# cts198859/deeprl_signal_control

Hardware: AMD Instinct MI355X
Metric: env-steps/s (agents x envs x sim-steps/s), large_grid MA2C (higher is better)
Workload: dtype f32; 1 GPU; large_grid 5x5 (25 agents), MA2C LSTM policy (neighbour fingerprint gather), 1024 env instances per GPU; step = 120 control steps (x5 sim-steps) of every instance + 1 A2C update (BPTT, clip, RMSProp); envs_per_gpu=1024, n_step=120, agents=25, parallelism=env-sharded x1, live_vehicles=window mean over the timed region

## Files before the change

### deeprl_signal_control_amd/csrc/tsc_model.hip

```cpp
#include "tsc_common.h"
#include "tsc_gemm.h"
#include "../../include/tsc.h"

#include <cstdlib>
#include <type_traits>
#include <vector>

namespace {

using tsc::f32x16;
using tsc::f32x4;
using tsc::GemmArgs;

constexpr int kOut = 8;
constexpr int kL = 64;
constexpr int kG4 = 4 * kL;

struct Layout {
    int G, A, SMAX, AMAX, H;
    int NZ, fc;
    long long stride, oW1, ob1, oWx, oWh, obl, oWo, obo;
};

__device__ __forceinline__ float sigmoidf_(float x) {
// ... 1632 lines not shown

__global__ void rmsprop_kernel(float *w, float *ms, const float *grad, long long per_agent, long long total,
                               const double *norm2, float gscale, float clip, float lr, float alpha, float eps) {
    const long long i = (long long)blockIdx.x * blockDim.x + threadIdx.x;
    if (i >= total) return;
    const int a = (int)(i / per_agent);
    const float nrm = (float)sqrt(norm2[a]);
    float g = grad[i] * gscale;
    if (clip > 0.f) g = g * (clip / fmaxf(nrm, clip));
    const float m = alpha * ms[i] + (1.0f - alpha) * g * g;
    ms[i] = m;
    w[i] = w[i] - lr * g / sqrtf(m + eps);
}

__global__ void transpose_wx_kernel(const float *params, Layout lay, float *WxT) {
    const long long i = (long long)blockIdx.x * blockDim.x + threadIdx.x;
    const long long per = (long long)lay.H * lay.NZ;
    if (i >= per * lay.G) return;
    const int g = (int)(i / per);
    const long long r = i % per;
    const int c = (int)(r / lay.H), h = (int)(r % lay.H);
    WxT[i] = params[(long long)g * lay.stride + lay.oWx + (long long)h * lay.NZ + c];
}

__global__ void interleave_gates_kernel(const float *params, Layout lay, float *Wg) {
    const long long i = (long long)blockIdx.x * blockDim.x + threadIdx.x;
    const long long per = (long long)(lay.H + kL) * kG4;
    if (i >= per * lay.G) return;
    const long long g = i / per, r = i % per;
    const int k = (int)(r / kG4), c = (int)(r % kG4), u = c >> 2, q = c & 3;
    Wg[i] = params[g * lay.stride + lay.oWx + (long long)k * kG4 + 64 * q + u];
}

__global__ void register_order_kernel(const float *params, Layout lay, float *Wr) {
    const long long i = (long long)blockIdx.x * blockDim.x + threadIdx.x;
    const long long per = (long long)(lay.H + kL) * kG4;
    if (i >= per * lay.G) return;
    const long long g = i / per, r = i % per;
    const int c = (int)(r & 3), lane = (int)((r >> 2) & 63);
    const long long rest = r >> 8;
    const int nj = (lay.H + kL) / 8, w = (int)(rest / nj), j4 = (int)(rest % nj);
    const int k = 8 * j4 + 4 * (lane >> 5) + c, col = 32 * w + (lane & 31);
    Wr[i] = params[g * lay.stride + lay.oWx + (long long)k * kG4 + col];
}

__global__ void fill_kernel(float *p, long long n, float v) {
    const long long i = (long long)blockIdx.x * blockDim.x + threadIdx.x;
    if (i < n) p[i] = v;
}

}


template <int NT>
__global__ void __launch_bounds__(512, 1)
dwxh_kernel(const float *__restrict__ X1, const float *__restrict__ Hp, const float *__restrict__ dZ, long long N, int G,
            int S, long long rows_per_split, float *__restrict__ ws) {
    constexpr int HT = NT - 2, H = 32 * HT, KC = 16, LDA = NT * 32 + 4;
    constexpr int XQ = H / 4, NX = KC * XQ, NQ = NX + KC * (kL / 4), NLD = (NQ + 511) / 512;
    __shared__ __attribute__((aligned(16))) float As[2][KC][LDA];
    const int g = blockIdx.x % G, sp = blockIdx.x / G;
    const int tid = threadIdx.x, lane = tid & 63, wave = tid >> 6, li = lane & 31, kh = lane >> 5;
    const int col0 = 32 * wave;
    const long long n0 = (long long)sp * rows_per_split;
    long long n1 = n0 + rows_per_split;
    if (n1 > N) n1 = N;
    const float *x1 = X1 + (long long)g * N * H, *hp = Hp + (long long)g * N * kL;
    const float *dz = dZ + (long long)g * N * kG4 + col0 + li;
    f32x16 acc[NT];
#pragma unroll
    for (int t = 0; t < NT; ++t)
#pragma unroll
        for (int r = 0; r < 16; ++r) acc[t][r] = 0.f;
    float bsum = 0.f;
    static_assert(NLD <= 3, "staging slots");
    struct Slot { int row, col; bool x, ok; };
    auto slot = [&](int q) {
        Slot o;
        int idx = tid + 512 * q;
        o.ok = idx < NQ;
        if (!o.ok) idx = NQ - 1;
        o.x = idx < NX;
        const int j = o.x ? idx : idx - NX, w = o.x ? XQ : kL / 4;
        o.row = j / w; o.col = 4 * (j % w);
        return o;
    };
    const Slot s0 = slot(0), s1 = slot(1), s2 = slot(2);
    float4 g0, g1, g2;
    auto fetch1 = [&](const Slot &o, long long row0) {
        long long row = row0 + o.row;
        if (row >= n1) row = n1 - 1;
        const float *src = o.x ? x1 + row * H + o.col : hp + row * kL + o.col;
        return *reinterpret_cast<const float4 *>(src);
    };
    auto commit1 = [&](const Slot &o, int buf, const float4 &v) {
        if (o.ok) *reinterpret_cast<float4 *>(&As[buf][o.row][(o.x ? 0 : H) + o.col]) = v;
    };
#define DWXH_FETCH(row0) do { g0 = fetch1(s0, row0); if (NLD > 1) g1 = fetch1(s1, row0); if (NLD > 2) g2 = fetch1(s2, row0); } while (0)
#define DWXH_COMMIT(buf) do { commit1(s0, buf, g0); if (NLD > 1) commit1(s1, buf, g1); if (NLD > 2) commit1(s2, buf, g2); } while (0)
    float bcur[KC / 2], bnxt[KC / 2];
    auto fetch_b = [&](float *b, long long row0) {
#pragma unroll
        for (int ks = 0; ks < KC / 2; ++ks) {
            const long long row = row0 + 2 * ks + kh;
            const float z = dz[(row < n1 ? row : n1 - 1) * kG4];
            b[ks] = row < n1 ? z : 0.f;
        }
    };
    if (n0 < n1) {
        DWXH_FETCH(n0); fetch_b(bcur, n0);
        DWXH_COMMIT(0);
        DWXH_FETCH(n0 + KC);
        __syncthreads();
        int buf = 0;
        for (long long row = n0; row < n1; row += KC, buf ^= 1) {
            fetch_b(bnxt, row + KC);
            __builtin_amdgcn_sched_barrier(0);
#pragma unroll
            for (int ks = 0; ks < KC / 2; ++ks) {
                float av[NT];
#pragma unroll
                for (int t = 0; t < NT; ++t) av[t] = As[buf][2 * ks + kh][32 * t + li];
                bsum += bcur[ks];
#pragma unroll
                for (int t = 0; t < NT; ++t) acc[t] = __builtin_amdgcn_mfma_f32_32x32x2f32(av[t], bcur[ks], acc[t], 0, 0, 0);
            }
            __builtin_amdgcn_sched_barrier(0);
            DWXH_COMMIT(buf ^ 1);
            DWXH_FETCH(row + 2 * KC);
#pragma unroll
            for (int ks = 0; ks < KC / 2; ++ks) bcur[ks] = bnxt[ks];
            __syncthreads();
        }
    }
    float *w = ws + ((long long)sp * G + g) * ((long long)(NT * 32 + 1) * kG4);
#pragma unroll
    for (int t = 0; t < NT; ++t)
#pragma unroll
        for (int r = 0; r < 16; ++r) {
            const int row = 32 * t + (r & 3) + 8 * (r >> 2) + 4 * kh;
            w[(long long)row * kG4 + col0 + li] = acc[t][r];
        }
    bsum += __shfl_xor(bsum, 32, 64);
    if (kh == 0) w[(long long)NT * 32 * kG4 + col0 + li] = bsum;
#undef DWXH_FETCH
#undef DWXH_COMMIT
}

__global__ void dwxh_reduce_kernel(const float *__restrict__ ws, int G, int S, long long per, float *__restrict__ grads,
                                   long long stride, long long off) {
    const long long i = (long long)blockIdx.x * blockDim.x + threadIdx.x;
    if (i >= per * G) return;
    const long long g = i / per, j = i % per;
    float acc = 0.f;
    for (int s = 0; s < S; ++s) acc += ws[((long long)s * G + g) * per + j];
    grads[g * stride + off + j] = acc;
}


constexpr int kD1Ld = 260;
constexpr int kObLd = 68;

template <int NCU>
__global__ void __launch_bounds__(512, 1)
dx1w1_kernel2(const float *__restrict__ dZ, const float *__restrict__ X1, const float *__restrict__ WxT,
              const float *__restrict__ obs, long long N, int G, int S, long long rows_per_split, int A, int SMAX,
              float *__restrict__ ws, const int *__restrict__ ftm) {
    constexpr int H = 16 * NCU, NHU = 2 * NCU;
    constexpr int CHI = (NHU + 7) / 8, CLO = NHU / 8;
    static_assert(NHU % 8 == 0 || NHU % 8 == 4, "H must be a multiple of 32");
    extern __shared__ __attribute__((aligned(16))) char smem_raw[];
    float *Az = (float *)smem_raw;
    float *Ob = Az + 2 * 32 * kD1Ld;
    const int g = blockIdx.x % G, sp = blockIdx.x / G, a = g >> 1;
    const int tid = threadIdx.x, lane = tid & 63, wave = __builtin_amdgcn_readfirstlane(tid >> 6), n = lane & 15, kq = lane >> 4;
    const long long n0 = (long long)sp * rows_per_split;
    long long n1 = n0 + rows_per_split;
    if (n1 > N) n1 = N;
    const float *dz = dZ + (long long)g * N * kG4, *x1 = X1 + (long long)g * N * H;
    const long long AS = (long long)A * SMAX;
    const int sq = SMAX >> 2;
    float *w = ws + ((long long)sp * G + g) * ((long long)2 * 65 * H);
    const int st = wave < 4 ? wave * CHI : 4 * CHI + (wave - 4) * CLO, cnt = wave < 4 ? CHI : CLO;
    const int U0 = st >> 1;
    const bool a00 = 2 * U0 >= st, a01 = 2 * U0 + 1 < st + cnt, a10 = 2 * U0 + 2 < st + cnt, a11 = 2 * U0 + 3 < st + cnt;
    const int U1 = U0 + 1 < NCU ? U0 + 1 : NCU - 1;
    const int col0 = 16 * U0 + n, col1 = 16 * U1 + n;
    const int fm0 = ftm[a * NCU + U0], fm1 = ftm[a * NCU + U1];
    float bw0[64], bw1[64];
    {
        const float *src = WxT + (long long)g * kG4 * H + (long long)(4 * kq) * H;
#pragma unroll
        for (int j = 0; j < 16; ++j)
#pragma unroll
            for (int c = 0; c < 4; ++c) {
                bw0[4 * j + c] = src[(long long)(16 * j + c) * H + col0];
                bw1[4 * j + c] = src[(long long)(16 * j + c) * H + col1];
            }
    }
    f32x4 accW[2][4];
#pragma unroll
    for (int u = 0; u < 2; ++u)
#pragma unroll
        for (int ft = 0; ft < 4; ++ft) accW[u][ft] = f32x4{0.f, 0.f, 0.f, 0.f};
    float bsum0 = 0.f, bsum1 = 0.f;
    const int zr = tid >> 6, zc = tid & 63, orow = tid >> 4, oc = tid & 15;
    float4 s0, s1, s2, s3, so;
    auto fetch = [&](long long row0) {
        auto rowc = [&](long long r) { return r < n1 ? r : n1 - 1; };
        s0 = *reinterpret_cast<const float4 *>(dz + rowc(row0 + zr) * kG4 + 4 * zc);
        s1 = *reinterpret_cast<const float4 *>(dz + rowc(row0 + zr + 8) * kG4 + 4 * zc);
        s2 = *reinterpret_cast<const float4 *>(dz + rowc(row0 + zr + 16) * kG4 + 4 * zc);
        s3 = *reinterpret_cast<const float4 *>(dz + rowc(row0 + zr + 24) * kG4 + 4 * zc);
        const float4 o = *reinterpret_cast<const float4 *>(obs + rowc(row0 + orow) * AS + (long long)a * SMAX + 4 * (oc < sq ? oc : 0));
        so = oc < sq ? o : make_float4(0.f, 0.f, 0.f, 0.f);
    };
    auto put = [&](int buf) {
        float *zb = Az + (long long)buf * 32 * kD1Ld + 4 * zc;
        *reinterpret_cast<float4 *>(zb + (zr) * kD1Ld) = s0;
        *reinterpret_cast<float4 *>(zb + (zr + 8) * kD1Ld) = s1;
        *reinterpret_cast<float4 *>(zb + (zr + 16) * kD1Ld) = s2;
        *reinterpret_cast<float4 *>(zb + (zr + 24) * kD1Ld) = s3;
        *reinterpret_cast<float4 *>(Ob + ((long long)buf * 32 + orow) * kObLd + 4 * oc) = so;
    };
    auto unit = [&](int buf, long long row, const float (&bw)[64], int col, bool r0, bool r1, f32x4 (&aw)[4], float &bs, int fm) {
        float xm0[4], xm1[4];
        int zq = 0;
        asm volatile("" : "+v"(zq));
#pragma unroll
        for (int i = 0; i < 4; ++i) {
            long long ra = row + 4 * kq + i + zq, rb = ra + 16;
            if (ra >= n1) ra = n1 - 1;
            if (rb >= n1) rb = n1 - 1;
            xm0[i] = x1[ra * H + col];
            xm1[i] = x1[rb * H + col];
        }
        f32x4 c0 = f32x4{0.f, 0.f, 0.f, 0.f}, c1 = f32x4{0.f, 0.f, 0.f, 0.f};
        const float4 *A0 = reinterpret_cast<const float4 *>(Az + ((long long)buf * 32 + n) * kD1Ld + 4 * kq);
        const float4 *A1 = reinterpret_cast<const float4 *>(Az + ((long long)buf * 32 + 16 + n) * kD1Ld + 4 * kq);
        if (r0 && r1) {
            float4 p = A0[0], q = A1[0];
#pragma unroll
            for (int j = 0; j < 16; ++j) {
                const float4 pn = A0[4 * (j + 1 < 16 ? j + 1 : j)], qn = A1[4 * (j + 1 < 16 ? j + 1 : j)];
                c0 = __builtin_amdgcn_mfma_f32_16x16x4f32(p.x, bw[4 * j], c0, 0, 0, 0);
                c1 = __builtin_amdgcn_mfma_f32_16x16x4f32(q.x, bw[4 * j], c1, 0, 0, 0);
                c0 = __builtin_amdgcn_mfma_f32_16x16x4f32(p.y, bw[4 * j + 1], c0, 0, 0, 0);
                c1 = __builtin_amdgcn_mfma_f32_16x16x4f32(q.y, bw[4 * j + 1], c1, 0, 0, 0);
                c0 = __builtin_amdgcn_mfma_f32_16x16x4f32(p.z, bw[4 * j + 2], c0, 0, 0, 0);
                c1 = __builtin_amdgcn_mfma_f32_16x16x4f32(q.z, bw[4 * j + 2], c1, 0, 0, 0);
                c0 = __builtin_amdgcn_mfma_f32_16x16x4f32(p.w, bw[4 * j + 3], c0, 0, 0, 0);
                c1 = __builtin_amdgcn_mfma_f32_16x16x4f32(q.w, bw[4 * j + 3], c1, 0, 0, 0);
                p = pn; q = qn;
                __builtin_amdgcn_sched_barrier(0);
            }
        } else {
            const float4 *As = r0 ? A0 : A1;
            float4 p = As[0];
#pragma unroll
            for (int j = 0; j < 16; ++j) {
                const float4 pn = As[4 * (j + 1 < 16 ? j + 1 : j)];
                c0 = __builtin_amdgcn_mfma_f32_16x16x4f32(p.x, bw[4 * j], c0, 0, 0, 0);
                c0 = __builtin_amdgcn_mfma_f32_16x16x4f32(p.y, bw[4 * j + 1], c0, 0, 0, 0);
                c0 = __builtin_amdgcn_mfma_f32_16x16x4f32(p.z, bw[4 * j + 2], c0, 0, 0, 0);
                c0 = __builtin_amdgcn_mfma_f32_16x16x4f32(p.w, bw[4 * j + 3], c0, 0, 0, 0);
                p = pn;
                __builtin_amdgcn_sched_barrier(0);
            }
            if (!r0) { c1 = c0; }
        }
        auto tail = [&](int r, const f32x4 &c, const float (&xm)[4]) {
            const float *Os = Ob + ((long long)buf * 32 + 16 * r + 4 * kq) * kObLd + n;
            float os[16];
#pragma unroll
            for (int i = 0; i < 4; ++i)
#pragma unroll
                for (int ft = 0; ft < 4; ++ft) os[4 * ft + i] = Os[i * kObLd + 16 * ft];
            float d[4];
#pragma unroll
            for (int i = 0; i < 4; ++i) {
                d[i] = (xm[i] > 0.f && row + 16 * r + 4 * kq + i < n1) ? c[i] : 0.f;
                bs += d[i];
            }
#pragma unroll
            for (int ft = 0; ft < 4; ++ft)
                if ((fm >> ft) & 1) {
#pragma unroll
                    for (int i = 0; i < 4; ++i) aw[ft] = __builtin_amdgcn_mfma_f32_16x16x4f32(os[4 * ft + i], d[i], aw[ft], 0, 0, 0);
                }
        };
        if (r0) tail(0, c0, xm0);
        if (r1) tail(1, c1, xm1);
    };
    if (n0 < n1) {
        fetch(n0);
        put(0);
        __syncthreads();
        int buf = 0;
        for (long long row = n0; row < n1; row += 32, buf ^= 1) {
            fetch(row + 32);
            if (a00 || a01) unit(buf, row, bw0, col0, a00, a01, accW[0], bsum0, fm0);
            if (a10 || a11) unit(buf, row, bw1, col1, a10, a11, accW[1], bsum1, fm1);
            put(buf ^ 1);
            __syncthreads();
        }
    }
    auto flush = [&](const f32x4 (&aw)[4], float bs, int col, bool r0, bool r1) {
        float *w0 = w + (long long)((r0 ? 0 : 1) * 65) * H;
        float *wz = w + (long long)65 * H;
#pragma unroll
        for (int ft = 0; ft < 4; ++ft)
#pragma unroll
            for (int i = 0; i < 4; ++i) {
                const int f = 16 * ft + 4 * kq + i;
                w0[(long long)f * H + col] = aw[ft][i];
                if (r0 && r1) wz[(long long)f * H + col] = 0.f;
            }
        bs += __shfl_xor(bs, 16, 64);
        bs += __shfl_xor(bs, 32, 64);
        if (kq == 0) {
            w0[(long long)64 * H + col] = bs;
            if (r0 && r1) wz[(long long)64 * H + col] = 0.f;
        }
    };
    if (a00 || a01) flush(accW[0], bsum0, col0, a00, a01);
    if (a10 || a11) flush(accW[1], bsum1, col1, a10, a11);
}

__global__ void dx1w1_reduce2_kernel(const float *__restrict__ ws, int G, int S, int H, int SMAX, const int16_t *__restrict__ rr,
                                     float *__restrict__ grads, long long stride, long long oW1, long long ob1) {
    const long long per = (long long)65 * H, out = (long long)(SMAX + 1) * H;
    const long long i = (long long)blockIdx.x * blockDim.x + threadIdx.x;
    if (i >= out * G) return;
    const long long g = i / out, j = i % out;
    const int f = (int)(j / H), n = (int)(j % H);
    const long long src = f < SMAX ? j : (long long)64 * H + n;
    float acc = 0.f;
    for (int s = 0; s < S; ++s) {
        acc += ws[(((long long)s * G + g) * 2 + 0) * per + src];
        acc += ws[(((long long)s * G + g) * 2 + 1) * per + src];
    }
    if (f < SMAX) {
        const int16_t *q = rr + ((g >> 1) * SMAX + f) * 2;
        if (n < q[0] || n >= q[1]) acc = 0.f;
        grads[g * stride + oW1 + j] = acc;
    } else {
        grads[g * stride + ob1 + n] = acc;
    }
}

constexpr int kFbLdz = kL + 4;

template <int NCU>
__global__ void __launch_bounds__(512, 1)
fc_bwd_kernel(const float *__restrict__ dZ, const float *__restrict__ X1, const float *__restrict__ WxT,
              const float *__restrict__ obs, long long N, int G, int S, long long rows_per_split, int A, int SMAX,
              float *__restrict__ ws, const int *__restrict__ ftm) {
    constexpr int H = 16 * NCU, NHU = 2 * NCU;
    constexpr int CHI = (NHU + 7) / 8, CLO = NHU / 8;
// ... 357 lines not shown
        TSC_HIP(m->bufs.upload(&m->krange, kr.data(), kr.size()));
    }
    {
        const int ncu = (L.H + 15) / 16;
        std::vector<int> fm((size_t)L.A * ncu, 0);
        for (int a = 0; a < L.A; ++a)
            for (int u = 0; u < ncu; ++u)
                for (int j = 0; j < L.SMAX && j < 64; ++j) {
                    const int lo = rr[((size_t)a * L.SMAX + j) * 2], hi = rr[((size_t)a * L.SMAX + j) * 2 + 1];
                    if (lo < 16 * u + 16 && hi > 16 * u) fm[(size_t)a * ncu + u] |= 1 << (j >> 4);
                }
        TSC_HIP(m->bufs.upload(&m->ftmask, fm.data(), fm.size()));
    }
    TSC_HIP(m->bufs.upload(&m->n_act, cfg->n_act, L.A));
    const long long E = n_env, T = m->T, N = E * T, G = L.G, A = L.A;
    TSC_HIP(m->bufs.alloc(&m->params, m->nparam, true)); TSC_HIP(m->bufs.alloc(&m->grads, m->nparam, true)); TSC_HIP(m->bufs.alloc(&m->ms, m->nparam, true));
    TSC_HIP(m->bufs.alloc(&m->WxT, G * L.H * kG4, true));
    TSC_HIP(m->bufs.alloc(&m->Wg, G * (L.H + kL) * kG4, true));
    m->wg_dirty = 1;
    TSC_HIP(m->bufs.alloc(&m->state_fw, G * E * 2 * kL, true)); TSC_HIP(m->bufs.alloc(&m->state_bw, G * E * 2 * kL, true));
    TSC_HIP(m->bufs.alloc(&m->r_obs, (N + E) * A * L.SMAX, true));
    TSC_HIP(m->bufs.alloc(&m->r_act, N * A, true)); TSC_HIP(m->bufs.alloc(&m->r_rew, N * A, true));
    TSC_HIP(m->bufs.alloc(&m->r_val, N * A, true)); TSC_HIP(m->bufs.alloc(&m->r_done, (T + 1) * E, true));
    TSC_HIP(m->bufs.alloc(&m->Rs, N * A, true)); TSC_HIP(m->bufs.alloc(&m->Advs, N * A, true));
    TSC_HIP(m->bufs.alloc(&m->X1, G * N * L.H + 32 * L.H, true));
    TSC_HIP(m->bufs.alloc(&m->Z, G * N * kG4, true));
    TSC_HIP(m->bufs.alloc(&m->Hh, G * N * kL, true)); TSC_HIP(m->bufs.alloc(&m->Cc, G * N * kL, true)); TSC_HIP(m->bufs.alloc(&m->Hp, G * N * kL, true));
    TSC_HIP(m->bufs.alloc(&m->dHh, G * N * kL, true));
    TSC_HIP(m->bufs.alloc(&m->norm2, A, true)); TSC_HIP(m->bufs.alloc(&m->stats, A * 6, true));
    TSC_HIP(m->bufs.alloc(&m->norm_part, A * kNormParts, true));
    m->logp_old = nullptr; m->ppo_ready = 0;
    m->ws_floats = (size_t)48 << 20; m->wsc_floats = (size_t)1 << 20;
    TSC_HIP(m->bufs.alloc(&m->ws, m->ws_floats, true)); TSC_HIP(m->bufs.alloc(&m->wsc, m->wsc_floats, true));
    m->lds_fwd = sizeof(float) * (64 * kWhLd + 64 * kHsLd);
    m->lds_fused = sizeof(float) * ((size_t)(L.H + 64) * kXLd + kL * kOut + kOut + 8);
    m->lds_ws = sizeof(float) * ((size_t)32 * (L.H + 64 + 4) + 64 * kWsLdx + (size_t)kL * kWsLdg + (size_t)kG4 * kWsLdg + 528 + (kWsBuf + 2) * 32 * kOut + (size_t)L.SMAX * L.H);
    m->dbg = nullptr;
    m->cached_next = 0;
    m->inplace = 0;

    const auto env_int = [](const char *name, int unset) { const char *ev = getenv(name); return ev ? atoi(ev) : unset; };
    const char *fwd_ws = getenv("TSC_FWD_WS");
    const bool unfused_dx = env_int("TSC_UNFUSED_DX", 0) != 0;
    m->dbg_tid = env_int("TSC_DBG_THREAD", 0);
    Plan &P = m->plan;
    P.s_upd = 256 / (int)G;
    if (P.s_upd < 1) P.s_upd = 1;
    P.s_fwd = P.s_upd < (E + 31) / 32 ? P.s_upd : (int)((E + 31) / 32);
    const bool wide = with_fused_width(L.H, [](auto) {}), narrow_obs = L.SMAX <= 64;
    const auto ws_fits = [&](long long per_split) { return (size_t)(P.s_upd * G * per_split) <= m->ws_floats; };
    if (!L.fc) {
        const bool tile = L.H % 32 == 0 && narrow_obs && m->lds_fused <= kLdsMax;
        P.fwd = !tile ? Fwd::Dense : wide && m->lds_ws <= kLdsMax && !(fwd_ws && fwd_ws[0] == '0') ? Fwd::Ws : Fwd::Tile;
        P.dwxh = wide && !env_int("TSC_UNFUSED_DW", 0) && ws_fits((long long)(L.H + kL + 1) * kG4);
        P.dx1w1 = wide && narrow_obs && !unfused_dx && ws_fits((long long)2 * 65 * L.H);
    } else {
        P.fwd = wide && narrow_obs && env_int("TSC_FC_MFMA", 1) ? Fwd::FcMfma
              : L.H % 16 == 0 && narrow_obs && fc_thread_lds(L.H) <= kLdsMax ? Fwd::FcThread : Fwd::Dense;
        P.fc_bwd = wide && narrow_obs && !unfused_dx && ws_fits((long long)2 * 65 * L.H + (long long)(L.H + 1) * kL);
    }
    m->fwd_wgs = (unsigned)(G * P.s_fwd);
    if (P.fwd == Fwd::Ws && env_int("TSC_FWD_XCD", 1) && P.s_fwd > 1 && P.s_fwd < 256) {
        const int S = P.s_fwd, cap = (L.G * S + 7) / 8;
        std::vector<int> tab((size_t)8 * cap, -1), used(8, 0);
        for (int gg = 0; gg < L.G; ++gg) {
            int left = S, spn = 0;
            while (left > 0) {
                int x = 0;
                for (int k = 1; k < 8; ++k) if (cap - used[k] > cap - used[x]) x = k;
                const int take = left < cap - used[x] ? left : cap - used[x];
                for (int q = 0; q < take; ++q) tab[(size_t)(used[x] + q) * 8 + x] = (gg << 8) | (spn + q);
                used[x] += take; spn += take; left -= take;
            }
        }
        TSC_HIP(m->bufs.upload(&m->wgmap, tab.data(), tab.size()));
        m->fwd_wgs = (unsigned)tab.size();
    }
    hipError_t attr = hipSuccess;
    const auto allow_lds = [&attr](const void *k) {
        if (attr == hipSuccess) attr = hipFuncSetAttribute(k, hipFuncAttributeMaxDynamicSharedMemorySize, (int)kLdsMax);
    };
    allow_lds((const void *)lstm_bwd2_kernel);
    allow_lds((const void *)lstm_fwd_kernel<true>);
    allow_lds((const void *)lstm_fwd_kernel<false>);
    if (P.fwd == Fwd::Tile) allow_lds((const void *)policy_fwd_fused_kernel);
    if (P.fwd == Fwd::FcThread) allow_lds((const void *)policy_fwd_fc_kernel);
    with_fused_width(L.H, [&](auto w) {
        constexpr int H = decltype(w)::value;
        if (P.fwd == Fwd::Ws) allow_lds((const void *)policy_fwd_ws_kernel<(H + kL) / 2>);
        if (P.fwd == Fwd::FcMfma) allow_lds((const void *)policy_fwd_fc_mfma_kernel<H / 32>);
        if (P.dx1w1) allow_lds((const void *)dx1w1_kernel2<H / 16>);
        if (P.fc_bwd) allow_lds((const void *)fc_bwd_kernel<H / 16>);
    });
    TSC_HIP(attr);
    hipLaunchKernelGGL(fill_kernel, dim3((unsigned)((m->nparam + 255) / 256)), dim3(256), 0, 0, m->ms, m->nparam, 1.0f);
    TSC_HIP(hipDeviceSynchronize());
    *out = guard.release();
    return 0;
}

int tsc_model_destroy(tsc_model *m) {
    if (!m) return 0;
    (void)hipSetDevice(m->device);
    delete m;
    return 0;
}

int tsc_model_set_stream(tsc_model *m, void *s) {
    if (!m) return tsc::fail("null handle");
    m->stream = (hipStream_t)s;
    return 0;
}

int tsc_model_layout(tsc_model *m, int64_t out[12]) {
    if (!m || !out) return tsc::fail("tsc_model_layout: bad arguments");
    const Layout &L = m->lay;
    const int64_t v[12] = {L.G, L.stride, L.H, kL, L.oW1, L.ob1, L.oWx, L.oWh, L.obl, L.oWo, L.obo, kOut};
    for (int i = 0; i < 12; ++i) out[i] = v[i];
    return 0;
}

int tsc_model_set_params(tsc_model *m, const float *h) {
    if (!m || !h) return tsc::fail("tsc_model_set_params: bad arguments");
    m->cached_next = -1;
    m->ppo_ready = 0;
    m->wg_dirty = 1;
    TSC_HIP(hipStreamSynchronize(m->stream));
    TSC_HIP(hipMemcpy(m->params, h, sizeof(float) * m->nparam, hipMemcpyHostToDevice));
    return 0;
}
int tsc_model_reset_opt_state(tsc_model *m) {
    if (!m) return tsc::fail("null handle");
    hipLaunchKernelGGL(fill_kernel, dim3((unsigned)((m->nparam + 255) / 256)), dim3(256), 0, m->stream, m->ms, m->nparam, 1.0f);
    TSC_HIP(hipGetLastError());
    TSC_HIP(hipStreamSynchronize(m->stream));
    return 0;
}
int tsc_model_get_params(tsc_model *m, float *h) {
    if (!m || !h) return tsc::fail("tsc_model_get_params: bad arguments");
    TSC_HIP(hipStreamSynchronize(m->stream));
    TSC_HIP(hipMemcpy(h, m->params, sizeof(float) * m->nparam, hipMemcpyDeviceToHost));
    return 0;
}
// ... 223 lines not shown
        tsc::ProfScope ps9(tsc::KID_TRANSPOSE, m->stream);
        hipLaunchKernelGGL(transpose_wx_kernel, dim3((unsigned)((G * L.H * L.NZ + 255) / 256)), dim3(256), 0, st, m->params, L, m->WxT);
        ps9.stop();
        TSC_HIP(hipGetLastError());
        if (P.fc_bwd) {
            long long rps = (N + S - 1) / S;
            rps = (rps + 31) / 32 * 32;
            const size_t lds = sizeof(float) * (2 * 32 * kFbLdz + 2 * 32 * kObLd + 2 * 32 * (L.H + 16));
            {
                tsc::ProfScope ps(tsc::KID_DX1_GEMM, m->stream);
                with_fused_width(L.H, [&](auto w) {
                    hipLaunchKernelGGL(fc_bwd_kernel<decltype(w)::value / 16>, dim3((unsigned)(S * G)), dim3(512), lds, st, m->dHh, m->X1,
                                       m->WxT, m->r_obs, N, (int)G, S, rps, (int)A, L.SMAX, m->ws, m->ftmask);
                });
            }
            {
                tsc::ProfScope ps(tsc::KID_DW1_GEMM, m->stream);
                const long long tot = ((long long)(L.SMAX + 1) * L.H + (long long)(L.H + 1) * kL) * G;
                hipLaunchKernelGGL(fc_bwd_reduce_kernel, dim3((unsigned)((tot + 255) / 256)), dim3(256), 0, st, m->ws, (int)G, S, L.H, L.SMAX,
                                   m->rowrange, g, L.stride, L.oW1, L.ob1, L.oWx);
            }
            TSC_HIP(hipGetLastError());
            m->cached_next = 0;
            return 0;
        }
        if (gemm(m, tsc::KID_DWX_GEMM, true, tsc::EPI_NONE, (int)G, L.H, kL, (int)N, m->X1, N * L.H, L.H, 1, m->dHh, N * kL, kL, g + L.oWx,
                 L.stride, kL, nullptr, 0, nullptr, 0, 0, nullptr, 0, g + L.obl, L.stride)) return tsc::fail("gemm failed");
        if (gemm(m, tsc::KID_DX1_GEMM, false, tsc::EPI_MASK_POS, (int)G, (int)N, L.H, kL, m->dHh, N * kL, kL, 1, m->WxT, (long long)L.H * kL, L.H,
                 m->X1, N * L.H, L.H, nullptr, 0, m->X1, N * L.H, L.H, nullptr, 0, nullptr, 0)) return tsc::fail("gemm failed");
    } else {
    if (m->cached_next != (int)T) {
        if (dense_forward(m, m->r_obs, N, m->X1, m->Z)) return tsc::fail("gemm launch failed");
        tsc::ProfScope ps2(tsc::KID_LSTM_FWD, m->stream);
        hipLaunchKernelGGL(lstm_fwd_kernel<true>, dim3((unsigned)G, (unsigned)((E + 63) / 64)), dim3(256), m->lds_fwd, st, m->params, L,
                           m->Z, m->state_bw, (float *)nullptr, m->Hh, m->Cc, m->Hp, m->r_done, (int)T, (int)E, 1);
        ps2.stop();
    }
    if (launch_head_bwd(m, N, beta, ppo)) return tsc::fail("head_bwd failed");
    tsc::ProfScope ps8(tsc::KID_LSTM_BWD, m->stream);
    hipLaunchKernelGGL(lstm_bwd2_kernel, dim3((unsigned)G, (unsigned)((E + 31) / 32)), dim3(256), sizeof(float) * 32 * (kDz2Ld + kDh3Ld), st,
                       m->params, L, m->Z, m->Cc, m->state_bw, m->dHh, m->r_done, (int)T, (int)E);
    ps8.stop();
    tsc::ProfScope ps9(tsc::KID_TRANSPOSE, m->stream);
    hipLaunchKernelGGL(transpose_wx_kernel, dim3((unsigned)((G * L.H * kG4 + 255) / 256)), dim3(256), 0, st, m->params, L, m->WxT);
    ps9.stop();
    TSC_HIP(hipGetLastError());
    if (P.dwxh) {
        const long long per = (long long)(L.H + kL + 1) * kG4;
        long long rps = (N + S - 1) / S;
        rps += rps & 1;
        {
            tsc::ProfScope ps(tsc::KID_DWX_GEMM, m->stream);
            with_fused_width(L.H, [&](auto w) {
                hipLaunchKernelGGL(dwxh_kernel<(decltype(w)::value + kL) / 32>, dim3((unsigned)(S * G)), dim3(512), 0, st, m->X1, m->Hp,
                                   m->Z, N, (int)G, S, rps, m->ws);
            });
        }
        {
            tsc::ProfScope ps(tsc::KID_DWH_GEMM, m->stream);
            hipLaunchKernelGGL(dwxh_reduce_kernel, dim3((unsigned)((per * G + 255) / 256)), dim3(256), 0, st, m->ws, (int)G, S, per, g,
                               L.stride, L.oWx);
        }
        TSC_HIP(hipGetLastError());
    } else {
    if (gemm(m, tsc::KID_DWH_GEMM, true, tsc::EPI_NONE, (int)G, kL, kG4, (int)N, m->Hp, N * kL, kL, 1, m->Z, N * kG4, kG4, g + L.oWh, L.stride,
             kG4, nullptr, 0, nullptr, 0, 0, nullptr, 0, g + L.obl, L.stride)) return tsc::fail("gemm failed");
    if (gemm(m, tsc::KID_DWX_GEMM, true, tsc::EPI_NONE, (int)G, L.H, kG4, (int)N, m->X1, N * L.H, L.H, 1, m->Z, N * kG4, kG4, g + L.oWx, L.stride,
             kG4, nullptr, 0, nullptr, 0, 0, nullptr, 0, nullptr, 0)) return tsc::fail("gemm failed");
    }
    if (P.dx1w1) {
        long long rps = (N + S - 1) / S;
        rps = (rps + 31) / 32 * 32;
        const size_t lds = sizeof(float) * (2 * 32 * kD1Ld + 2 * 32 * kObLd);
        {
            tsc::ProfScope ps(tsc::KID_DX1_GEMM, m->stream);
            with_fused_width(L.H, [&](auto w) {
                hipLaunchKernelGGL(dx1w1_kernel2<decltype(w)::value / 16>, dim3((unsigned)(S * G)), dim3(512), lds, st, m->Z, m->X1, m->WxT,
                                   m->r_obs, N, (int)G, S, rps, (int)A, L.SMAX, m->ws, m->ftmask);
            });
        }
        {
            tsc::ProfScope ps(tsc::KID_DW1_GEMM, m->stream);
            const long long tot = (long long)(L.SMAX + 1) * L.H * G;
            hipLaunchKernelGGL(dx1w1_reduce2_kernel, dim3((unsigned)((tot + 255) / 256)), dim3(256), 0, st, m->ws, (int)G, S, L.H, L.SMAX,
                               m->rowrange, g, L.stride, L.oW1, L.ob1);
        }
        TSC_HIP(hipGetLastError());
        m->cached_next = 0;
        return 0;
    }
    if (gemm(m, tsc::KID_DX1_GEMM, false, tsc::EPI_MASK_POS, (int)G, (int)N, L.H, kG4, m->Z, N * kG4, kG4, 1, m->WxT, (long long)L.H * kG4, L.H,
             m->X1, N * L.H, L.H, nullptr, 0, m->X1, N * L.H, L.H, nullptr, 0, nullptr, 0)) return tsc::fail("gemm failed");
    }
    if (gemm(m, tsc::KID_DW1_GEMM, true, tsc::EPI_ROWRANGE, (int)G, L.SMAX, L.H, (int)N, m->r_obs, L.SMAX, AS, 2, m->X1, N * L.H, L.H, g + L.oW1,
             L.stride, L.H, nullptr, 0, nullptr, 0, 0, m->rowrange, L.SMAX, g + L.ob1, L.stride)) return tsc::fail("gemm failed");
    m->cached_next = 0;
    TSC_HIP(hipGetLastError());
    return 0;
}

int tsc_model_compute_grads(tsc_model *m, const float *R_boot, double beta) {
    if (!m || !R_boot) return tsc::fail("tsc_model_compute_grads: bad arguments");
    m->ppo_ready = 0;
    return compute_grads_impl(m, R_boot, beta, nullptr);
}

int tsc_model_compute_grads_ppo(tsc_model *m, const float *R_boot, double beta, double clip_eps, double gae_lambda, int32_t epoch) {
    if (!m || epoch < 0 || (epoch == 0 && !R_boot)) return tsc::fail("tsc_model_compute_grads_ppo: bad arguments");
    if (!(clip_eps > 0.0)) return tsc::fail("tsc_model_compute_grads_ppo: clip_eps %g must be positive", clip_eps);
    if (!(gae_lambda > 0.0 && gae_lambda <= 1.0)) return tsc::fail("tsc_model_compute_grads_ppo: gae_lambda %g outside (0, 1]", gae_lambda);
    if (epoch > 0 && !m->ppo_ready)
        return tsc::fail("tsc_model_compute_grads_ppo: epoch %d without epoch 0 on this rollout (advantages and logp_old are taken there)", epoch);
    if (!m->logp_old) {
        TSC_HIP(hipSetDevice(m->device));
        TSC_HIP(m->bufs.alloc(&m->logp_old, (size_t)m->T * m->E * m->lay.A, true));
    }
    const PpoArgs ppo = {clip_eps, gae_lambda, epoch};
    if (epoch == 0) m->ppo_ready = 0;
    if (compute_grads_impl(m, R_boot, beta, &ppo)) return 1;
    m->ppo_ready = 1;
    return 0;
}

int tsc_model_ppo_stats(tsc_model *m, double *out_host) {
    if (!m || !out_host) return tsc::fail("tsc_model_ppo_stats: bad arguments");
    TSC_HIP(hipStreamSynchronize(m->stream));
    TSC_HIP(hipMemcpy(out_host, m->stats + 4 * m->lay.A, sizeof(double) * 2 * m->lay.A, hipMemcpyDeviceToHost));
    return 0;
}

int tsc_model_grad_buffer(tsc_model *m, float **grad, int64_t *count) {
// ... 104 lines not shown
```

Before: 384.6 million env-steps/s.

## Deepen dwxh LDS pipeline to 8 stages and split clamp/plain load paths

The dW_x/dW_h gradient kernel moves from a 2-buffer static LDS stage to an 8-slot dynamic-LDS ring. Fetches run four chunks ahead, and a barrier is issued only every four chunks, with staging split between lead and trailing waves around the MFMA block. Both dwxh and dx1w1 gain an unclamped fast path that uses wave-uniform (readfirstlane) global base pointers and 32-bit offsets for interior chunks, keeping clamped addressing only for the tail. The aim is to hide global load latency and cut address arithmetic and synchronisation, at the cost of much more LDS, which is now gated by an LDS-size check. Optional clock64 timing stamps are added behind a compile flag.

```diff
diff --git a/deeprl_signal_control_amd/csrc/tsc_model.hip b/deeprl_signal_control_amd/csrc/tsc_model.hip
--- a/deeprl_signal_control_amd/csrc/tsc_model.hip
+++ b/deeprl_signal_control_amd/csrc/tsc_model.hip
@@ -1708,87 +1708,139 @@
 }
 
 
+typedef const float __attribute__((address_space(1))) *gfloat_p;
+typedef const f32x4 __attribute__((address_space(1))) *gfloat4_p;
+__device__ __forceinline__ gfloat_p uniform_ptr(const float *p) {
+    const unsigned long long v = (unsigned long long)p;
+    const unsigned lo = __builtin_amdgcn_readfirstlane((unsigned)v), hi = __builtin_amdgcn_readfirstlane((unsigned)(v >> 32));
+    return (gfloat_p)(((unsigned long long)hi << 32) | lo);
+}
+
+constexpr int kDwKc = 16, kDwKi = 64;
+template <int NT> constexpr size_t dwxh_lds() { return sizeof(float) * 2 * kDwKi * (NT * 32 + 4); }
+
 template <int NT>
 __global__ void __launch_bounds__(512, 1)
 dwxh_kernel(const float *__restrict__ X1, const float *__restrict__ Hp, const float *__restrict__ dZ, long long N, int G,
-            int S, long long rows_per_split, float *__restrict__ ws) {
-    constexpr int HT = NT - 2, H = 32 * HT, KC = 16, LDA = NT * 32 + 4;
-    constexpr int XQ = H / 4, NX = KC * XQ, NQ = NX + KC * (kL / 4), NLD = (NQ + 511) / 512;
-    __shared__ __attribute__((aligned(16))) float As[2][KC][LDA];
+            int S, long long rows_per_split, float *__restrict__ ws, long long *dbg) {
+    constexpr int HT = NT - 2, H = 32 * HT, KC = kDwKc, LDA = NT * 32 + 4;
+    constexpr int XQ = H / 4, NX = KC * XQ;
+    static_assert(NX >= 512 && NX <= 1024 && NX % 64 == 0 && KC * (kL / 4) == 256, "staging slots");
+    extern __shared__ __attribute__((aligned(16))) char smem_raw[];
+    float *As = (float *)smem_raw;
     const int g = blockIdx.x % G, sp = blockIdx.x / G;
-    const int tid = threadIdx.x, lane = tid & 63, wave = tid >> 6, li = lane & 31, kh = lane >> 5;
+    const int tid = threadIdx.x, lane = tid & 63, wave = __builtin_amdgcn_readfirstlane(tid >> 6), li = lane & 31, kh = lane >> 5;
     const int col0 = 32 * wave;
     const long long n0 = (long long)sp * rows_per_split;
     long long n1 = n0 + rows_per_split;
     if (n1 > N) n1 = N;
+    const long long R = n1 - n0;
     const float *x1 = X1 + (long long)g * N * H, *hp = Hp + (long long)g * N * kL;
-    const float *dz = dZ + (long long)g * N * kG4 + col0 + li;
+    const float *dz = dZ + (long long)g * N * kG4;
     f32x16 acc[NT];
 #pragma unroll
     for (int t = 0; t < NT; ++t)
 #pragma unroll
         for (int r = 0; r < 16; ++r) acc[t][r] = 0.f;
     float bsum = 0.f;
-    static_assert(NLD <= 3, "staging slots");
-    struct Slot { int row, col; bool x, ok; };
-    auto slot = [&](int q) {
-        Slot o;
-        int idx = tid + 512 * q;
-        o.ok = idx < NQ;
-        if (!o.ok) idx = NQ - 1;
-        o.x = idx < NX;
-        const int j = o.x ? idx : idx - NX, w = o.x ? XQ : kL / 4;
-        o.row = j / w; o.col = 4 * (j % w);
-        return o;
+    const bool has1 = wave < (NX - 512) / 64, has2 = wave >= 4;
+    struct Slots { int r0, c0, r1, c1, r2, c2; };
+    auto slots = [&](int t) {
+        const int i1 = has1 ? t + 512 : t, i2 = t & 255;
+        return Slots{t / XQ, 4 * (t % XQ), i1 / XQ, 4 * (i1 % XQ), i2 >> 4, 4 * (i2 & 15)};
     };
-    const Slot s0 = slot(0), s1 = slot(1), s2 = slot(2);
-    float4 g0, g1, g2;
-    auto fetch1 = [&](const Slot &o, long long row0) {
-        long long row = row0 + o.row;
-        if (row >= n1) row = n1 - 1;
-        const float *src = o.x ? x1 + row * H + o.col : hp + row * kL + o.col;
-        return *reinterpret_cast<const float4 *>(src);
+    const Slots sl = slots(tid);
+    const unsigned o0 = sl.r0 * H + sl.c0, o1 = sl.r1 * H + sl.c1, o2 = sl.r2 * kL + sl.c2;
+    const unsigned l0 = sl.r0 * LDA + sl.c0, l1 = sl.r1 * LDA + sl.c1, l2 = sl.r2 * LDA + H + sl.c2;
+    const unsigned zb = kh * kG4 + col0 + li;
+    f32x4 g0, g1, g2;
+    float bcur[KC / 2], bnxt[KC / 2];
+    using Clamp = std::true_type;
+    using Plain = std::false_type;
+    auto fetch_a = [&](auto cl, long long c) {
+        if constexpr (decltype(cl)::value) {
+            int t = tid;
+            asm volatile("" : "+v"(t));
+            const Slots q = slots(t);
+            auto rowc = [&](long long r) { return r < n1 ? r : n1 - 1; };
+            const long long b = n0 + KC * c;
+            g0 = *reinterpret_cast<const f32x4 *>(x1 + rowc(b + q.r0) * H + q.c0);
+            if (has1) g1 = *reinterpret_cast<const f32x4 *>(x1 + rowc(b + q.r1) * H + q.c1);
+            if (has2) g2 = *reinterpret_cast<const f32x4 *>(hp + rowc(b + q.r2) * kL + q.c2);
+        } else {
+            const gfloat_p xs = uniform_ptr(x1 + (n0 + KC * c) * H), hs = uniform_ptr(hp + (n0 + KC * c) * kL);
+            g0 = *(gfloat4_p)(xs + o0);
+            if (has1) g1 = *(gfloat4_p)(xs + o1);
+            if (has2) g2 = *(gfloat4_p)(hs + o2);
+        }
     };
-    auto commit1 = [&](const Slot &o, int buf, const float4 &v) {
-        if (o.ok) *reinterpret_cast<float4 *>(&As[buf][o.row][(o.x ? 0 : H) + o.col]) = v;
+    auto commit_a = [&](long long c) {
+        float *d = As + (unsigned)(c & 7) * (KC * LDA);
+        *reinterpret_cast<f32x4 *>(d + l0) = g0;
+        if (has1) *reinterpret_cast<f32x4 *>(d + l1) = g1;
+        if (has2) *reinterpret_cast<f32x4 *>(d + l2) = g2;
     };
-#define DWXH_FETCH(row0) do { g0 = fetch1(s0, row0); if (NLD > 1) g1 = fetch1(s1, row0); if (NLD > 2) g2 = fetch1(s2, row0); } while (0)
-#define DWXH_COMMIT(buf) do { commit1(s0, buf, g0); if (NLD > 1) commit1(s1, buf, g1); if (NLD > 2) commit1(s2, buf, g2); } while (0)
-    float bcur[KC / 2], bnxt[KC / 2];
-    auto fetch_b = [&](float *b, long long row0) {
+    auto fetch_b = [&](auto cl, float *b, long long c) {
+        if constexpr (decltype(cl)::value) {
+#pragma unroll
+            for (int ks = 0; ks < KC / 2; ++ks) {
+                const long long row = n0 + KC * c + 2 * ks + kh;
+                const float z = dz[((row < n1 ? row : n1 - 1) - kh) * kG4 + zb];
+                b[ks] = row < n1 ? z : 0.f;
+            }
+        } else {
+            const gfloat_p zs = uniform_ptr(dz + (n0 + KC * c) * kG4);
+#pragma unroll
+            for (int ks = 0; ks < KC / 2; ++ks) b[ks] = (zs + 2 * ks * kG4)[zb];
+        }
+    };
+#ifdef TSC_UPD_STAMPS
+    long long *stp = dbg && blockIdx.x == 0 && (tid == 0 || tid == 256) ? dbg + (tid >> 8) * 8 : nullptr;
+#define USTAMP(k, cc) do { if (stp && (cc) == 11) stp[k] = clock64(); } while (0)
+#else
+#define USTAMP(k, cc) do { } while (0)
+#endif
+    const bool lead = wave < 4;
+    auto sub = [&](auto cl, long long c) {
+        USTAMP(0, c);
+        auto stage = [&]() { commit_a(c + 4); fetch_a(cl, c + 5); };
+        fetch_b(cl, bnxt, c + 1);
+        if (lead) stage();
+        const float *a = As + (unsigned)(c & 7) * (KC * LDA) + kh * LDA + li;
+        __builtin_amdgcn_sched_barrier(0);
+        USTAMP(1, c);
 #pragma unroll
         for (int ks = 0; ks < KC / 2; ++ks) {
-            const long long row = row0 + 2 * ks + kh;
-            const float z = dz[(row < n1 ? row : n1 - 1) * kG4];
-            b[ks] = row < n1 ? z : 0.f;
-        }
+            float av[NT];
+#pragma unroll
+            for (int t = 0; t < NT; ++t) av[t] = a[2 * ks * LDA + 32 * t];
+            bsum += bcur[ks];
+#pragma unroll
+            for (int t = 0; t < NT; ++t) acc[t] = __builtin_amdgcn_mfma_f32_32x32x2f32(av[t], bcur[ks], acc[t], 0, 0, 0);
+        }
+        USTAMP(2, c);
+        __builtin_amdgcn_sched_barrier(0);
+        if (!lead) stage();
+#pragma unroll
+        for (int ks = 0; ks < KC / 2; ++ks) bcur[ks] = bnxt[ks];
+        USTAMP(3, c);
     };
-    if (n0 < n1) {
-        DWXH_FETCH(n0); fetch_b(bcur, n0);
-        DWXH_COMMIT(0);
-        DWXH_FETCH(n0 + KC);
+    if (R > 0) {
+        for (int c = 0; c < 4; ++c) { fetch_a(Clamp{}, c); commit_a(c); }
+        fetch_a(Clamp{}, 4); fetch_b(Clamp{}, bcur, 0);
         __syncthreads();
-        int buf = 0;
-        for (long long row = n0; row < n1; row += KC, buf ^= 1) {
-            fetch_b(bnxt, row + KC);
-            __builtin_amdgcn_sched_barrier(0);
-#pragma unroll
-            for (int ks = 0; ks < KC / 2; ++ks) {
-                float av[NT];
-#pragma unroll
-                for (int t = 0; t < NT; ++t) av[t] = As[buf][2 * ks + kh][32 * t + li];
-                bsum += bcur[ks];
-#pragma unroll
-                for (int t = 0; t < NT; ++t) acc[t] = __builtin_amdgcn_mfma_f32_32x32x2f32(av[t], bcur[ks], acc[t], 0, 0, 0);
-            }
-            __builtin_amdgcn_sched_barrier(0);
-            DWXH_COMMIT(buf ^ 1);
-            DWXH_FETCH(row + 2 * KC);
-#pragma unroll
-            for (int ks = 0; ks < KC / 2; ++ks) bcur[ks] = bnxt[ks];
+        long long c = 0;
+        for (; KC * (c + 9) <= R; c += 4) {
+            sub(Plain{}, c); sub(Plain{}, c + 1); sub(Plain{}, c + 2); sub(Plain{}, c + 3);
             __syncthreads();
-        }
-    }
+            USTAMP(4, c + 3);
+        }
+        for (; KC * c < R; ++c) {
+            sub(Clamp{}, c);
+            if ((c & 3) == 3) __syncthreads();
+        }
+    }
+#undef USTAMP
     float *w = ws + ((long long)sp * G + g) * ((long long)(NT * 32 + 1) * kG4);
 #pragma unroll
     for (int t = 0; t < NT; ++t)
@@ -1799,8 +1851,6 @@
         }
     bsum += __shfl_xor(bsum, 32, 64);
     if (kh == 0) w[(long long)NT * 32 * kG4 + col0 + li] = bsum;
-#undef DWXH_FETCH
-#undef DWXH_COMMIT
 }
 
 __global__ void dwxh_reduce_kernel(const float *__restrict__ ws, int G, int S, long long per, float *__restrict__ grads,
@@ -1821,7 +1871,7 @@
 __global__ void __launch_bounds__(512, 1)
 dx1w1_kernel2(const float *__restrict__ dZ, const float *__restrict__ X1, const float *__restrict__ WxT,
               const float *__restrict__ obs, long long N, int G, int S, long long rows_per_split, int A, int SMAX,
-              float *__restrict__ ws, const int *__restrict__ ftm) {
+              float *__restrict__ ws, const int *__restrict__ ftm, long long *dbg) {
     constexpr int H = 16 * NCU, NHU = 2 * NCU;
     constexpr int CHI = (NHU + 7) / 8, CLO = NHU / 8;
     static_assert(NHU % 8 == 0 || NHU % 8 == 4, "H must be a multiple of 32");
@@ -1861,35 +1911,60 @@
         for (int ft = 0; ft < 4; ++ft) accW[u][ft] = f32x4{0.f, 0.f, 0.f, 0.f};
     float bsum0 = 0.f, bsum1 = 0.f;
     const int zr = tid >> 6, zc = tid & 63, orow = tid >> 4, oc = tid & 15;
-    float4 s0, s1, s2, s3, so;
-    auto fetch = [&](long long row0) {
-        auto rowc = [&](long long r) { return r < n1 ? r : n1 - 1; };
-        s0 = *reinterpret_cast<const float4 *>(dz + rowc(row0 + zr) * kG4 + 4 * zc);
-        s1 = *reinterpret_cast<const float4 *>(dz + rowc(row0 + zr + 8) * kG4 + 4 * zc);
-        s2 = *reinterpret_cast<const float4 *>(dz + rowc(row0 + zr + 16) * kG4 + 4 * zc);
-        s3 = *reinterpret_cast<const float4 *>(dz + rowc(row0 + zr + 24) * kG4 + 4 * zc);
-        const float4 o = *reinterpret_cast<const float4 *>(obs + rowc(row0 + orow) * AS + (long long)a * SMAX + 4 * (oc < sq ? oc : 0));
-        so = oc < sq ? o : make_float4(0.f, 0.f, 0.f, 0.f);
+    f32x4 s0, s1, s2, s3, so;
+    using Clamp = std::true_type;
+    using Plain = std::false_type;
+    const unsigned zo = zr * kG4 + 4 * zc, oo = (unsigned)orow * (unsigned)AS + 4 * (oc < sq ? oc : 0);
+    const bool ob_ok = oc < sq;
+    auto fetch = [&](auto cl, long long row0) {
+        if constexpr (decltype(cl)::value) {
+            auto rowc = [&](long long r) { return r < n1 ? r : n1 - 1; };
+            s0 = *reinterpret_cast<const f32x4 *>(dz + rowc(row0 + zr) * kG4 + 4 * zc);
+            s1 = *reinterpret_cast<const f32x4 *>(dz + rowc(row0 + zr + 8) * kG4 + 4 * zc);
+            s2 = *reinterpret_cast<const f32x4 *>(dz + rowc(row0 + zr + 16) * kG4 + 4 * zc);
+            s3 = *reinterpret_cast<const f32x4 *>(dz + rowc(row0 + zr + 24) * kG4 + 4 * zc);
+            const f32x4 o = *reinterpret_cast<const f32x4 *>(obs + rowc(row0 + orow) * AS + (long long)a * SMAX + 4 * (oc < sq ? oc : 0));
+            so = ob_ok ? o : f32x4{0.f, 0.f, 0.f, 0.f};
+        } else {
+            const gfloat_p zs = uniform_ptr(dz + row0 * kG4), os = uniform_ptr(obs + row0 * AS + (long long)a * SMAX);
+            s0 = *(gfloat4_p)(zs + zo);
+            s1 = *(gfloat4_p)(zs + 8 * kG4 + zo);
+            s2 = *(gfloat4_p)(zs + 16 * kG4 + zo);
+            s3 = *(gfloat4_p)(zs + 24 * kG4 + zo);
+            const f32x4 o = *(gfloat4_p)(os + oo);
+            so = ob_ok ? o : f32x4{0.f, 0.f, 0.f, 0.f};
+        }
     };
     auto put = [&](int buf) {
         float *zb = Az + (long long)buf * 32 * kD1Ld + 4 * zc;
-        *reinterpret_cast<float4 *>(zb + (zr) * kD1Ld) = s0;
-        *reinterpret_cast<float4 *>(zb + (zr + 8) * kD1Ld) = s1;
-        *reinterpret_cast<float4 *>(zb + (zr + 16) * kD1Ld) = s2;
-        *reinterpret_cast<float4 *>(zb + (zr + 24) * kD1Ld) = s3;
-        *reinterpret_cast<float4 *>(Ob + ((long long)buf * 32 + orow) * kObLd + 4 * oc) = so;
+        *reinterpret_cast<f32x4 *>(zb + (zr) * kD1Ld) = s0;
+        *reinterpret_cast<f32x4 *>(zb + (zr + 8) * kD1Ld) = s1;
+        *reinterpret_cast<f32x4 *>(zb + (zr + 16) * kD1Ld) = s2;
+        *reinterpret_cast<f32x4 *>(zb + (zr + 24) * kD1Ld) = s3;
+        *reinterpret_cast<f32x4 *>(Ob + ((long long)buf * 32 + orow) * kObLd + 4 * oc) = so;
     };
-    auto unit = [&](int buf, long long row, const float (&bw)[64], int col, bool r0, bool r1, f32x4 (&aw)[4], float &bs, int fm) {
+    auto unit = [&](auto cl, int buf, long long row, const float (&bw)[64], int col, bool r0, bool r1, f32x4 (&aw)[4], float &bs, int fm) {
+        constexpr bool clamp = decltype(cl)::value;
         float xm0[4], xm1[4];
         int zq = 0;
         asm volatile("" : "+v"(zq));
-#pragma unroll
-        for (int i = 0; i < 4; ++i) {
-            long long ra = row + 4 * kq + i + zq, rb = ra + 16;
-            if (ra >= n1) ra = n1 - 1;
-            if (rb >= n1) rb = n1 - 1;
-            xm0[i] = x1[ra * H + col];
-            xm1[i] = x1[rb * H + col];
+        if constexpr (clamp) {
+#pragma unroll
+            for (int i = 0; i < 4; ++i) {
+                long long ra = row + 4 * kq + i + zq, rb = ra + 16;
+                if (ra >= n1) ra = n1 - 1;
+                if (rb >= n1) rb = n1 - 1;
+                xm0[i] = x1[ra * H + col];
+                xm1[i] = x1[rb * H + col];
+            }
+        } else {
+            const gfloat_p xs = uniform_ptr(x1 + row * H);
+            const unsigned xo = (unsigned)(4 * kq * H + col + zq);
+#pragma unroll
+            for (int i = 0; i < 4; ++i) {
+                xm0[i] = (xs + i * H)[xo];
+                xm1[i] = (xs + (16 + i) * H)[xo];
+            }
         }
         f32x4 c0 = f32x4{0.f, 0.f, 0.f, 0.f}, c1 = f32x4{0.f, 0.f, 0.f, 0.f};
         const float4 *A0 = reinterpret_cast<const float4 *>(Az + ((long long)buf * 32 + n) * kD1Ld + 4 * kq);
@@ -1935,7 +2010,7 @@
             float d[4];
 #pragma unroll
             for (int i = 0; i < 4; ++i) {
-                d[i] = (xm[i] > 0.f && row + 16 * r + 4 * kq + i < n1) ? c[i] : 0.f;
+                d[i] = (xm[i] > 0.f && (!clamp || row + 16 * r + 4 * kq + i < n1)) ? c[i] : 0.f;
                 bs += d[i];
             }
 #pragma unroll
@@ -1948,19 +2023,36 @@
         if (r0) tail(0, c0, xm0);
         if (r1) tail(1, c1, xm1);
     };
+#ifdef TSC_UPD_STAMPS
+    long long *stp = dbg && blockIdx.x == 0 && (tid == 0 || tid == 256) ? dbg + 16 + (tid >> 8) * 8 : nullptr;
+#define USTAMP(k) do { if (stp && row == n0 + 5 * 32) stp[k] = clock64(); } while (0)
+#else
+#define USTAMP(k) do { } while (0)
+#endif
+    const bool lead = wave < 4 || !(a10 || a11);
+    auto chunk = [&](auto cl, int buf, long long row) {
+        USTAMP(0);
+        if (lead) fetch(cl, row + 32);
+        USTAMP(1);
+        if (a00 || a01) unit(cl, buf, row, bw0, col0, a00, a01, accW[0], bsum0, fm0);
+        if (!lead) fetch(cl, row + 32);
+        if (a10 || a11) unit(cl, buf, row, bw1, col1, a10, a11, accW[1], bsum1, fm1);
+        USTAMP(2);
+        put(buf ^ 1);
+        USTAMP(3);
+        __syncthreads();
+        USTAMP(4);
+    };
     if (n0 < n1) {
-        fetch(n0);
+        fetch(Clamp{}, n0);
         put(0);
         __syncthreads();
         int buf = 0;
-        for (long long row = n0; row < n1; row += 32, buf ^= 1) {
-            fetch(row + 32);
-            if (a00 || a01) unit(buf, row, bw0, col0, a00, a01, accW[0], bsum0, fm0);
-            if (a10 || a11) unit(buf, row, bw1, col1, a10, a11, accW[1], bsum1, fm1);
-            put(buf ^ 1);
-            __syncthreads();
-        }
-    }
+        long long row = n0;
+        for (; row + 64 <= n1; row += 32, buf ^= 1) chunk(Plain{}, buf, row);
+        for (; row < n1; row += 32, buf ^= 1) chunk(Clamp{}, buf, row);
+    }
+#undef USTAMP
     auto flush = [&](const f32x4 (&aw)[4], float bs, int col, bool r0, bool r1) {
         float *w0 = w + (long long)((r0 ? 0 : 1) * 65) * H;
         float *wz = w + (long long)65 * H;
@@ -2424,7 +2516,9 @@
     if (!L.fc) {
         const bool tile = L.H % 32 == 0 && narrow_obs && m->lds_fused <= kLdsMax;
         P.fwd = !tile ? Fwd::Dense : wide && m->lds_ws <= kLdsMax && !(fwd_ws && fwd_ws[0] == '0') ? Fwd::Ws : Fwd::Tile;
-        P.dwxh = wide && !env_int("TSC_UNFUSED_DW", 0) && ws_fits((long long)(L.H + kL + 1) * kG4);
+        size_t lds_dwxh = 0;
+        with_fused_width(L.H, [&](auto w) { lds_dwxh = dwxh_lds<(decltype(w)::value + kL) / 32>(); });
+        P.dwxh = wide && lds_dwxh <= kLdsMax && !env_int("TSC_UNFUSED_DW", 0) && ws_fits((long long)(L.H + kL + 1) * kG4);
         P.dx1w1 = wide && narrow_obs && !unfused_dx && ws_fits((long long)2 * 65 * L.H);
     } else {
         P.fwd = wide && narrow_obs && env_int("TSC_FC_MFMA", 1) ? Fwd::FcMfma
@@ -2461,6 +2555,7 @@
         constexpr int H = decltype(w)::value;
         if (P.fwd == Fwd::Ws) allow_lds((const void *)policy_fwd_ws_kernel<(H + kL) / 2>);
         if (P.fwd == Fwd::FcMfma) allow_lds((const void *)policy_fwd_fc_mfma_kernel<H / 32>);
+        if (P.dwxh) allow_lds((const void *)dwxh_kernel<(H + kL) / 32>);
         if (P.dx1w1) allow_lds((const void *)dx1w1_kernel2<H / 16>);
         if (P.fc_bwd) allow_lds((const void *)fc_bwd_kernel<H / 16>);
     });
@@ -2790,8 +2885,9 @@
         {
             tsc::ProfScope ps(tsc::KID_DWX_GEMM, m->stream);
             with_fused_width(L.H, [&](auto w) {
-                hipLaunchKernelGGL(dwxh_kernel<(decltype(w)::value + kL) / 32>, dim3((unsigned)(S * G)), dim3(512), 0, st, m->X1, m->Hp,
-                                   m->Z, N, (int)G, S, rps, m->ws);
+                constexpr int NT = (decltype(w)::value + kL) / 32;
+                hipLaunchKernelGGL(dwxh_kernel<NT>, dim3((unsigned)(S * G)), dim3(512), dwxh_lds<NT>(), st, m->X1, m->Hp, m->Z, N, (int)G, S,
+                                   rps, m->ws, m->dbg);
             });
         }
         {
@@ -2814,7 +2910,7 @@
             tsc::ProfScope ps(tsc::KID_DX1_GEMM, m->stream);
             with_fused_width(L.H, [&](auto w) {
                 hipLaunchKernelGGL(dx1w1_kernel2<decltype(w)::value / 16>, dim3((unsigned)(S * G)), dim3(512), lds, st, m->Z, m->X1, m->WxT,
-                                   m->r_obs, N, (int)G, S, rps, (int)A, L.SMAX, m->ws, m->ftmask);
+                                   m->r_obs, N, (int)G, S, rps, (int)A, L.SMAX, m->ws, m->ftmask, m->dbg);
             });
         }
         {
```

Result: faster. 395.1 million env-steps/s, median of 6 (+2.8%).
